# NVlabs/WarpConvNet

Measured on AMD Instinct MI355X. Metric: M active voxels/sec fwd+bwd, SparseConv3d 64→128 k=3, 1/2/4/8 MI355X, higher is better.
Workload: dtype bf16; 1 GPU; configs[1]: one 1000000-voxel uniform (U) scene per GPU, SparseConv3d 64->128 k=3, bf16 autocast, kernel-map build + AB fwd + ABt dgrad + AtB wgrad per step; voxels_per_gpu=1000000, coord_order=generator, parallelism=dp1 (scene-sharded, grad all-reduce)

## Files before the change

warpconvnet_amd/csrc/kmap_binned.hip:

```cpp
#include "kmap_cells.h"

namespace wcn {

constexpr int kInsertSample = 8;
constexpr int kInsertThreads = 512;
constexpr int kRowBufPitch = 66;
constexpr int kRowBufInts = (kCompactPitch + 1) * kRowBufPitch;
#ifndef WCN_NB_WPE
#define WCN_NB_WPE 3
#endif
constexpr int kNbWavesPerSimd = WCN_NB_WPE;
constexpr int kNbThreads = 256;

__device__ __forceinline__ int wrap_blk(int v) {
  const int bits = kBlkCoordBits;
  v &= (1 << bits) - 1;
  return (v ^ (1 << (bits - 1))) - (1 << (bits - 1));
}

__global__ void cell_prepare_kernel(uint4* __restrict__ slots, int64_t capacity, int32_t* __restrict__ ctr,
                                    uint32_t* __restrict__ halo, CellGeom g, int32_t* __restrict__ status) {
  const int64_t i = (int64_t)blockIdx.x * blockDim.x + threadIdx.x;
  if (i < capacity) slots[i] = make_uint4(0u, 0u, 0xFFFFFFFFu, 0u);
  if (i < 64) ctr[i] = 0;
  if (i == 0) *status = 0;
  if (i < g.halo_cells) {
    const int h3[3] = {g.hx, g.hy, g.hz};
    int t = (int)i, dir = 0;
    int sx = 0, sy = 0, sz = 0;
    for (; dir < 27; ++dir) {
      if (dir == 13) continue;
      const int dd[3] = {dir / 9 - 1, (dir / 3) % 3 - 1, dir % 3 - 1};
      sx = dd[0] ? h3[0] : kBlk; sy = dd[1] ? h3[1] : kBlk; sz = dd[2] ? h3[2] : kBlk;
      const int cells = sx * sy * sz;
      if (t < cells) break;
      t -= cells;
    }
    const int ddx = dir / 9 - 1, ddy = (dir / 3) % 3 - 1, ddz = dir % 3 - 1;
    const int tz = t % sz, ty = (t / sz) % sy, tx = t / (sz * sy);
    const int lx = ddx < 0 ? kBlk - g.hx + tx : tx;
    const int ly = ddy < 0 ? kBlk - g.hy + ty : ty;
    const int lz = ddz < 0 ? kBlk - g.hz + tz : tz;
    const int X = lx + kBlk * ddx + g.hx, Y = ly + kBlk * ddy + g.hy, Z = lz + kBlk * ddz + g.hz;
    halo[i] = ((uint32_t)dir << 27) | ((uint32_t)cell_index(lx, ly, lz) << 16) | (uint32_t)(X * g.px + Y * g.py + Z);
  }
}

__device__ __forceinline__ void store_cell(int32_t* cell, int row, bool strict) {
  if (strict) __hip_atomic_fetch_min(reinterpret_cast<uint32_t*>(cell), (uint32_t)row, __ATOMIC_RELAXED, __HIP_MEMORY_SCOPE_AGENT);
  else *cell = row;
}

template <int PHASE>
__global__ __launch_bounds__(kInsertThreads) void cell_insert_kernel(BSlot* __restrict__ slots, uint32_t cmask,
                                                          const int4* __restrict__ coords, int64_t n, CellTable t,
                                                          int32_t* __restrict__ status, int kp, int mw,
                                                          int32_t* __restrict__ nbr, uint32_t* __restrict__ mask,
                                                          int strict) {
  const bool compact = kp < 0;
  kp &= 0x7FFFFFFF;
  const int64_t tid = (int64_t)blockIdx.x * blockDim.x + threadIdx.x;
  const int64_t i = PHASE == 0 ? tid * kInsertSample : tid;
  const int lane = threadIdx.x & 63;
  bool live = i < n;
  int4 c = make_int4(0, 0, 0, 0);
  if (live) {
    c = coords[i];
    if (!coord_in_range(c.x, c.y, c.z, c.w)) {
      live = false;
      if (PHASE == 1) {
        atomicOr(status, (int)WCN_FLAG_COORD_RANGE);
        for (int k = 0; k < kp; ++k) nbr[i * kp + k] = compact ? 0 : -1;
        for (int w = 0; w < mw; ++w) mask[i * mw + w] = 0u;
      }
    }
  }
  int found = -1;
  int id = -1;
  bool created = false;
  uint64_t key = 0;
  if (live) {
    key = pack_key(c.x, c.y >> kBlkShift, c.z >> kBlkShift, c.w >> kBlkShift);
    uint32_t s = hash_slot(key, cmask);
    int idv = -1;
    for (uint32_t a = 0; a <= cmask; ++a) {
      unsigned long long* kptr = reinterpret_cast<unsigned long long*>(&slots[s].key);
      const uint4 v = *reinterpret_cast<const uint4*>(slots + s);
      unsigned long long cur = ((unsigned long long)v.y << 32) | v.x;
      if (cur == key) { found = (int)s; idv = (int)v.z; break; }
      if (cur == 0ull) {
        if (PHASE == 1) cur = __hip_atomic_load(kptr, __ATOMIC_RELAXED, __HIP_MEMORY_SCOPE_AGENT);
        if (cur == 0ull) {
          cur = atomicCAS(kptr, 0ull, (unsigned long long)key);
          if (cur == 0ull) {
            created = true;
            found = (int)s;
            break;
          }
        }
        if (cur == key) { found = (int)s; break; }
      }
      s = (s + 1) & cmask;
    }
    if (found < 0) atomicOr(status, (int)WCN_FLAG_TABLE_FULL);
    if (PHASE == 1 && idv >= 0 && !(idv & kIdLateBit)) id = idv;
  }
  __shared__ int s_made[kInsertThreads / 64 + 1];
  const int wave = threadIdx.x >> 6;
  const unsigned long long makers = __ballot(created);
  if (PHASE == 0) {
    if (lane == 0) s_made[wave] = __popcll(makers);
    __syncthreads();
    if (threadIdx.x == 0) {
      int tot = 0;
      for (int w = 0; w < kInsertThreads / 64; ++w) {
        const int c = s_made[w];
        s_made[w] = tot;
        tot += c;
      }
      s_made[kInsertThreads / 64] = tot > 0 ? atomicAdd(&t.ctr[0], tot) : 0;
    }
    __syncthreads();
  }
  if (makers != 0ull) {
    int base;
    if (PHASE == 0) {
      base = s_made[kInsertThreads / 64] + s_made[wave];
    } else {
      const int leader = __ffsll((long long)makers) - 1;
      base = 0;
      if (lane == leader) base = atomicAdd(&t.ctr[0], __popcll(makers));
      base = __shfl(base, leader);
    }
    int my_id = base + __popcll(makers & ((1ull << lane) - 1ull));
    if (!created) my_id = -1;
    if (my_id >= t.max_blocks) {
      atomicOr(status, (int)WCN_FLAG_TABLE_FULL);
      my_id = -1;
    }
    if (my_id >= 0) {
      t.blk_key[my_id] = key;
      slots[found].id = my_id | (PHASE == 1 ? kIdLateBit : 0);
    }
    unsigned long long todo = makers;
    while (todo != 0ull) {
      const int src = __ffsll((long long)todo) - 1;
      todo &= todo - 1ull;
      const int bid = __shfl(my_id, src);
      if (bid >= 0) {
        int4* gcells = reinterpret_cast<int4*>(t.cells + (int64_t)bid * kCells);
        gcells[lane] = make_int4(-1, -1, -1, -1);
        gcells[lane + 64] = make_int4(-1, -1, -1, -1);
      }
    }
  }
  if (PHASE == 0) return;
  if (live) mask[i * mw + (mw - 1)] = (id >= 0 || found < 0) ? kMaskUnwritten : kMaskDeferred;
  if (id >= 0) store_cell(t.cells + (int64_t)id * kCells + cell_of(c), (int)i, strict != 0);
}

__global__ __launch_bounds__(256) void cell_finish_kernel(const BSlot* __restrict__ slots, uint32_t cmask,
                                                          const int4* __restrict__ coords, int64_t n, CellTable t,
                                                          CellGeom g, int mw, const uint32_t* __restrict__ mask,
                                                          int strict) {
  const int64_t tid = (int64_t)blockIdx.x * blockDim.x + threadIdx.x;
  const int64_t nthreads = (int64_t)gridDim.x * blockDim.x;
  for (int64_t i = tid; i < n; i += nthreads) {
    if (mask[i * mw + (mw - 1)] != kMaskDeferred) continue;
    const int4 c = coords[i];
    const int id = block_id_of(slots, cmask, c);
    if (id < 0) continue;
    store_cell(t.cells + (int64_t)id * kCells + cell_of(c), (int)i, strict != 0);
  }
  const int lane = threadIdx.x & 63;
  int nblocks = t.ctr[0];
  if (nblocks > t.max_blocks) nblocks = (int)t.max_blocks;
  for (int64_t seq = tid >> 6; seq < nblocks; seq += nthreads >> 6) {
    const int id = (int)seq;
    int nid = -1;
    if (lane < 27) {
      const int ddx = lane / 9 - 1, ddy = (lane / 3) % 3 - 1, ddz = lane % 3 - 1;
      const bool needed = (ddx == 0 || g.hx > 0) && (ddy == 0 || g.hy > 0) && (ddz == 0 || g.hz > 0);
      if (lane == 13) nid = id;
      else if (needed) {
        const uint64_t key = t.blk_key[id];
        const int b = (int)((key >> 54) & kBatchMask);
        const int bx = wrap_blk((int)((key >> 36) & kCoordMask));
        const int by = wrap_blk((int)((key >> 18) & kCoordMask));
        const int bz = wrap_blk((int)(key & kCoordMask));
        const int s = block_find(slots, cmask, pack_key(b, wrap_blk(bx + ddx), wrap_blk(by + ddy), wrap_blk(bz + ddz)));
        if (s >= 0) {
          nid = slots[s].id;
          if (nid >= 0) nid &= ~kIdLateBit;
        }
      }
    }
    if (lane < 32) t.nbtab[(int64_t)id * 32 + lane] = nid;
  }
}

#ifdef WCN_PROF
__device__ unsigned long long g_bprof[4096 * 12];
#define BSTAMP(i) do { const unsigned long long now_ = wall_clock64(); prof_acc[i] += now_ - prof_prev; prof_prev = now_; } while (0)
#else
#define BSTAMP(i)
#endif

template <int LPR, bool FAST, bool COMPACT>
__global__ __launch_bounds__(kNbThreads) __attribute__((amdgpu_waves_per_eu(kNbWavesPerSimd))) void cell_neighbors_kernel(CellTable t, const uint32_t* __restrict__ halo,
                                                                    CellGeom g, int K, int kp, int mw,
                                                                    int32_t* __restrict__ nbr,
                                                                    uint32_t* __restrict__ mask,
                                                                    int32_t* __restrict__ status) {
  extern __shared__ int s_mem[];
  const int lane = threadIdx.x & 63, wave = threadIdx.x >> 6;
  uint32_t* s_halo = reinterpret_cast<uint32_t*>(s_mem);
  const int rounds = (g.halo_cells + 63) >> 6;
  const bool halo_regs = COMPACT && rounds <= 8;
  const int halo_pad = halo_regs ? 0 : rounds * 64;
  const int per_wave = g.cells + 4 + kCells / 2 + 8 + (COMPACT ? kRowBufInts : 0);
  int* s_grid = s_mem + halo_pad + wave * per_wave;
  unsigned short* s_own = reinterpret_cast<unsigned short*>(s_grid + g.cells + 4);
  const int null_cell = g.cells;
  for (int h = threadIdx.x; h < halo_pad; h += blockDim.x) s_halo[h] = h < g.halo_cells ? halo[h] : 0xFFFFFFFFu;
  if (lane == 0) s_grid[null_cell] = -1;
  __syncthreads();

  int nblocks = t.ctr[0];
  if (nblocks > t.max_blocks) nblocks = (int)t.max_blocks;
  const int gwave = blockIdx.x * (blockDim.x / 64) + wave;
  const int nwaves = gridDim.x * (blockDim.x / 64);
  constexpr int kVoxPerIter = 64 / LPR;
  const int sub = lane % LPR, vsel = lane / LPR;
  const int num_chunks = (kp + LPR - 1) / LPR;
  uint32_t he[8];
#pragma unroll
  for (int u = 0; u < 8; ++u) {
    const int idx = u * 64 + lane;
    uint32_t e = COMPACT && idx < g.halo_cells ? halo[idx] : 0xFFFFFFFFu;
    if (e == 0xFFFFFFFFu) e = (31u << 27) | (uint32_t)(g.cells + 1);
    he[u] = e;
  }
  auto load_head = [&](int seq, int& nb, int4& v0, int4& v1) {
    nb = -1;
    v0 = make_int4(-1, -1, -1, -1);
    v1 = v0;
    if (seq < nblocks) {
      if (lane < 27) nb = t.nbtab[(int64_t)seq * 32 + lane];
      const int4* own = reinterpret_cast<const int4*>(t.cells + (int64_t)seq * kCells) + lane * 2;
      v0 = own[0];
      v1 = own[1];
    }
  };
  int seq = gwave;
  int nb_c, nb_n;
  int4 c0, c1, n0, n1;
  load_head(seq, nb_c, c0, c1);
  load_head(seq + nwaves, nb_n, n0, n1);
  int hv[8];
  auto gather = [&](int nb, int r0) {
#pragma unroll
    for (int u = 0; u < 8; ++u) {
      hv[u] = -1;
      if (r0 + u < rounds) {
        const uint32_t e = s_halo[(r0 + u) * 64 + lane];
        const int nid = __shfl(nb, (int)((e >> 27) & 31u));
        if (e != 0xFFFFFFFFu && nid >= 0) hv[u] = t.cells[(int64_t)nid * kCells + ((e >> 16) & (kCells - 1))];
      }
    }
  };
  int nidv[8];
  auto gather8 = [&](int nb) {
#pragma unroll
    for (int u = 0; u < 8; ++u) nidv[u] = __shfl(nb, (int)(he[u] >> 27));
#pragma unroll
    for (int u = 0; u < 8; ++u)
      if (u < rounds) {
        const int safe = nidv[u] < 0 ? 0 : nidv[u];
        hv[u] = t.cells[(int64_t)safe * kCells + ((he[u] >> 16) & (kCells - 1))];
      }
  };
  auto scatter8 = [&]() {
#pragma unroll
    for (int u = 0; u < 8; ++u)
      if (u < rounds) s_grid[he[u] & 0xFFFFu] = nidv[u] >= 0 ? hv[u] : -1;
  };
  auto scatter_halo = [&](int r0) {
#pragma unroll
    for (int u = 0; u < 8; ++u)
      if (r0 + u < rounds) {
        const uint32_t e = s_halo[(r0 + u) * 64 + lane];
        if (e != 0xFFFFFFFFu) s_grid[e & 0xFFFFu] = hv[u];
      }
  };
  int* s_rows = s_grid + g.cells + 4 + kCells / 2 + 8;
  int pend_row = -1;
  auto flush_rows = [&](int row) {
    __builtin_amdgcn_fence(__ATOMIC_RELEASE, "wavefront");
    __builtin_amdgcn_wave_barrier();
    if (row >= 0) mask[row] = (uint32_t)s_rows[lane];
    const int piece = lane & 3;
    int rid[4];
    int4 v[4];
#pragma unroll
    for (int q = 0; q < 4; ++q) rid[q] = __shfl(row, (lane >> 2) + 16 * q);
#pragma unroll
    for (int q = 0; q < 4; ++q) {
      const int r = (lane >> 2) + 16 * q;
      v[q].x = s_rows[(piece * 4 + 0) * kRowBufPitch + r];
      v[q].y = s_rows[(piece * 4 + 1) * kRowBufPitch + r];
      v[q].z = s_rows[(piece * 4 + 2) * kRowBufPitch + r];
      v[q].w = s_rows[(piece * 4 + 3) * kRowBufPitch + r];
    }
#pragma unroll
    for (int q = 0; q < 4; ++q)
      if (rid[q] >= 0 && __popc((uint32_t)s_rows[(lane >> 2) + 16 * q]) >= 4 * piece) {
        if (FAST)
          *reinterpret_cast<int4*>(reinterpret_cast<char*>(nbr) + (__umul24((uint32_t)rid[q], kCompactPitch * 4u) + (uint32_t)piece * 16u)) = v[q];
        else
          *reinterpret_cast<int4*>(nbr + (int64_t)rid[q] * kCompactPitch + piece * 4) = v[q];
      }
    __builtin_amdgcn_fence(__ATOMIC_ACQUIRE, "wavefront");
    __builtin_amdgcn_wave_barrier();
  };
#ifdef WCN_PROF
  if (lane == 0 && gwave < 4096) g_bprof[gwave * 12 + 9] = wall_clock64();
#endif
  if (seq < nblocks) {
    if (halo_regs) gather8(nb_c);
    else gather(nb_c, 0);
  }
#ifdef WCN_PROF
  unsigned long long prof_prev = wall_clock64(), prof_acc[8] = {0, 0, 0, 0, 0, 0, 0, 0}, prof_blocks = 0;
  const unsigned long long prof_loop0 = prof_prev;
#endif
  for (; seq < nblocks; seq += nwaves) {
    BSTAMP(0);
#ifdef WCN_PROF
    ++prof_blocks;
#endif
    if (halo_regs) scatter8();
    else scatter_halo(0);
    for (int r0 = 8; r0 < rounds; r0 += 8) {
      gather(nb_c, r0);
      scatter_halo(r0);
    }
    BSTAMP(1);
    const int vals[8] = {c0.x, c0.y, c0.z, c0.w, c1.x, c1.y, c1.z, c1.w};
    const int cell0 = ((lane >> 3) + g.hx) * g.px + ((lane & 7) + g.hy) * g.py + g.hz;
    int mine = 0;
#pragma unroll
    for (int z = 0; z < 8; ++z) {
      s_grid[cell0 + z] = vals[z];
      mine += vals[z] >= 0;
    }
    int incl = mine;
#pragma unroll
    for (int d = 1; d < 64; d <<= 1) {
      const int up = __shfl_up(incl, d);
      if (lane >= d) incl += up;
    }
    const int own_cnt = __shfl(incl, 63);
    int at = incl - mine;
#pragma unroll
    for (int z = 0; z < 8; ++z)
      if (vals[z] >= 0) s_own[at++] = (unsigned short)((cell0 + z) * 4);
    if (lane < 2 * kVoxPerIter) s_own[own_cnt + lane] = (unsigned short)(null_cell * 4);
    BSTAMP(4);
    if (COMPACT) {
      flush_rows(pend_row);
      pend_row = -1;
    }
    BSTAMP(5);
    nb_c = nb_n; c0 = n0; c1 = n1;
    if (seq + nwaves < nblocks) {
      if (halo_regs) gather8(nb_c);
      else gather(nb_c, 0);
    }
    BSTAMP(6);
    load_head(seq + 2 * nwaves, nb_n, n0, n1);
    __builtin_amdgcn_fence(__ATOMIC_RELEASE, "wavefront");
    __builtin_amdgcn_wave_barrier();
    BSTAMP(2);
    const char* grid_bytes = reinterpret_cast<const char*>(s_grid);
    if (COMPACT) {
      int delta_lane = 0;
      if (lane < K) {
        const int l = lane % g.kz, j = (lane / g.kz) % g.ky, i = lane / (g.kz * g.ky);
        delta_lane = ((i - g.cx) * g.dx * g.px + (j - g.cy) * g.dy * g.py + (l - g.cz) * g.dz) * 4;
      }
      bool over = false;
      char* rows_bytes = reinterpret_cast<char*>(s_rows);
      const int origin4 = (g.hx * g.px + g.hy * g.py + g.hz) * 4;
      const uint32_t wp0 = (uint32_t)(kRowBufPitch + lane) * 4u, wp_max = (uint32_t)(kCompactPitch * kRowBufPitch + lane) * 4u;
      for (int e0 = 0; e0 < own_cnt; e0 += 64) {
        const bool live = e0 + lane < own_cnt;
        const int cell = live ? (int)s_own[e0 + lane] : origin4;
        const int row = live ? *reinterpret_cast<const int*>(grid_bytes + cell) : -1;
        uint32_t wp = wp0, rev = 0;
        auto answer = [&](int f) {
          *reinterpret_cast<int*>(rows_bytes + wp) = f;
          const uint32_t h = f >= 0 ? 1u : 0u;
          rev = (rev << 1) | h;
          wp = min(wp + h * (uint32_t)(kRowBufPitch * 4), wp_max);
        };
        int k = 0;
        for (; k + 4 <= K; k += 4) {
          int f[4];
#pragma unroll
          for (int u = 0; u < 4; ++u)
            f[u] = *reinterpret_cast<const int*>(grid_bytes + cell + __builtin_amdgcn_readlane(delta_lane, k + u));
#pragma unroll
          for (int u = 0; u < 4; ++u) answer(f[u]);
        }
        for (; k < K; ++k) answer(*reinterpret_cast<const int*>(grid_bytes + cell + __builtin_amdgcn_readlane(delta_lane, k)));
        const uint32_t m = __brev(rev) >> (32 - K);
        over = over || (live && __popc(m) > kCompactIds);
        s_rows[lane] = (int)m;
        if (e0 + 64 < own_cnt) flush_rows(row);
        else pend_row = row;
      }
      if (__any(over) && lane == 0) atomicOr(status, (int)WCN_FLAG_ROW_OVERFLOW);
    } else
    for (int kc = 0; kc < num_chunks; ++kc) {
      const int k = kc * LPR + sub;
      const bool k_real = k < K, k_store = k < kp;
      const int l = k % g.kz, j = (k / g.kz) % g.ky, i = k / (g.kz * g.ky);
      const int ox = (i - g.cx) * g.dx, oy = (j - g.cy) * g.dy, oz = (l - g.cz) * g.dz;
      const int delta4 = k_real ? (ox * g.px + oy * g.py + oz) * 4 : 0;
      const int w0 = (kc * LPR) >> 5;
      for (int e0 = 0; e0 < own_cnt; e0 += 2 * kVoxPerIter) {
        const int cell_a = s_own[e0 + vsel], cell_b = s_own[e0 + kVoxPerIter + vsel];
        const int row_a = *reinterpret_cast<const int*>(grid_bytes + cell_a);
        const int row_b = *reinterpret_cast<const int*>(grid_bytes + cell_b);
        int found_a = *reinterpret_cast<const int*>(grid_bytes + cell_a + delta4);
        int found_b = *reinterpret_cast<const int*>(grid_bytes + cell_b + delta4);
        if (!k_real) { found_a = -1; found_b = -1; }
        const unsigned long long ball_a = __ballot(found_a >= 0), ball_b = __ballot(found_b >= 0);
        uint32_t bits_a, bits_b, hi_a = 0, hi_b = 0;
        if (LPR == 64) {
          bits_a = (uint32_t)ball_a; hi_a = (uint32_t)(ball_a >> 32);
          bits_b = (uint32_t)ball_b; hi_b = (uint32_t)(ball_b >> 32);
        } else if (LPR == 32) {
          bits_a = vsel ? (uint32_t)(ball_a >> 32) : (uint32_t)ball_a;
          bits_b = vsel ? (uint32_t)(ball_b >> 32) : (uint32_t)ball_b;
        } else {
          bits_a = (uint32_t)(ball_a >> (vsel * LPR)) & ((1u << LPR) - 1u);
          bits_b = (uint32_t)(ball_b >> (vsel * LPR)) & ((1u << LPR) - 1u);
        }
        if (FAST) {
          char* nbr_b = reinterpret_cast<char*>(nbr);
          char* mask_b = reinterpret_cast<char*>(mask);
          const uint32_t kp4 = (uint32_t)kp * 4u, mw4 = (uint32_t)mw * 4u, k4 = (uint32_t)k * 4u, w4 = (uint32_t)w0 * 4u;
          if (row_a >= 0 && k_store) *reinterpret_cast<int*>(nbr_b + (__umul24((uint32_t)row_a, kp4) + k4)) = found_a;
          if (row_b >= 0 && k_store) *reinterpret_cast<int*>(nbr_b + (__umul24((uint32_t)row_b, kp4) + k4)) = found_b;
          if (sub == 0 && w0 < mw) {
            if (row_a >= 0) *reinterpret_cast<uint32_t*>(mask_b + (__umul24((uint32_t)row_a, mw4) + w4)) = bits_a;
            if (row_b >= 0) *reinterpret_cast<uint32_t*>(mask_b + (__umul24((uint32_t)row_b, mw4) + w4)) = bits_b;
            if (LPR == 64 && w0 + 1 < mw) {
              if (row_a >= 0) *reinterpret_cast<uint32_t*>(mask_b + (__umul24((uint32_t)row_a, mw4) + w4 + 4u)) = hi_a;
              if (row_b >= 0) *reinterpret_cast<uint32_t*>(mask_b + (__umul24((uint32_t)row_b, mw4) + w4 + 4u)) = hi_b;
            }
          }
        } else {
          if (row_a >= 0 && k_store) nbr[(int64_t)row_a * kp + k] = found_a;
          if (row_b >= 0 && k_store) nbr[(int64_t)row_b * kp + k] = found_b;
          if (sub == 0 && w0 < mw) {
            if (row_a >= 0) mask[(int64_t)row_a * mw + w0] = bits_a;
            if (row_b >= 0) mask[(int64_t)row_b * mw + w0] = bits_b;
            if (LPR == 64 && w0 + 1 < mw) {
              if (row_a >= 0) mask[(int64_t)row_a * mw + w0 + 1] = hi_a;
              if (row_b >= 0) mask[(int64_t)row_b * mw + w0 + 1] = hi_b;
            }
          }
        }
      }
    }
    BSTAMP(3);

    __builtin_amdgcn_fence(__ATOMIC_ACQUIRE, "wavefront");
    __builtin_amdgcn_wave_barrier();
  }
  if (COMPACT) flush_rows(pend_row);
#ifdef WCN_PROF
  if (lane == 0 && gwave < 4096) {
    for (int i = 0; i < 8; ++i) g_bprof[gwave * 12 + i] = prof_acc[i];
    g_bprof[gwave * 12 + 8] = prof_blocks;
    g_bprof[gwave * 12 + 10] = prof_loop0;
    g_bprof[gwave * 12 + 11] = wall_clock64();
  }
#endif
}

static void launch_cell_table(const CellTable& t, const CellGeom& g, const int4* coords, int64_t n, int kp, int mw, int32_t* nbr,
                              uint32_t* mask, int32_t* status, int strict, hipStream_t s) {
  const int64_t capacity = t.capacity;
  const uint32_t cmask = (uint32_t)(capacity - 1);
  const int64_t max_blocks = t.max_blocks;
  const int64_t prep = capacity > g.halo_cells ? capacity : g.halo_cells;
  hipLaunchKernelGGL(cell_prepare_kernel, dim3((unsigned)ceil_div(prep, 256)), dim3(256), 0, s, (uint4*)t.slots, capacity,
                     t.ctr, t.halo, g, status);
  const int64_t n_first = ceil_div(n, kInsertSample);
  hipLaunchKernelGGL(cell_insert_kernel<0>, dim3((unsigned)ceil_div(n_first, kInsertThreads)), dim3(kInsertThreads), 0, s, t.slots, cmask,
                     coords, n, t, status, kp, mw, nbr, mask, strict);
  hipLaunchKernelGGL(cell_insert_kernel<1>, dim3((unsigned)ceil_div(n, kInsertThreads)), dim3(kInsertThreads), 0, s, t.slots, cmask,
                     coords, n, t, status, kp, mw, nbr, mask, strict);
  {
    const int64_t work = n > 64 * max_blocks ? n : 64 * max_blocks;
    int64_t wgs = ceil_div(work, 256);
    if (wgs > 8192) wgs = 8192;
    hipLaunchKernelGGL(cell_finish_kernel, dim3((unsigned)wgs), dim3(256), 0, s, (const BSlot*)t.slots, cmask,
                       coords, n, t, g, mw, (const uint32_t*)mask, strict);
  }
}

}

using namespace wcn;

extern "C" {

size_t wcn_kmap_binned_workspace(int64_t n, int64_t max_blocks) {
  if (n < 0) n = 0;
  if (max_blocks < 1) max_blocks = 1;
  return carve_cells(nullptr, n, max_blocks).bytes;
}

int wcn_kmap_binned_supported(const int32_t ksize[3], const int32_t dilation[3]) {
  if (!ksize || !dilation) return 0;
  for (int d = 0; d < 3; ++d) {
    if (ksize[d] < 1 || dilation[d] < 1) return 0;
  }
  const int32_t unit[3] = {1, 1, 1};
  const KernelGeom g = make_kernel_geom(ksize, unit, dilation);
  if (kernel_halo(g.kx, g.cx, g.dx) > kMaxHalo || kernel_halo(g.ky, g.cy, g.dy) > kMaxHalo ||
      kernel_halo(g.kz, g.cz, g.dz) > kMaxHalo)
    return 0;
  const int64_t K = (int64_t)ksize[0] * ksize[1] * ksize[2];
  return (valid_k(K) && (K & 31) != 0) ? 1 : 0;
}

int wcn_kmap_compact_supported(int32_t num_offsets) {
  return (num_offsets >= 17 && num_offsets <= 31) ? 1 : 0;
}

int wcn_kmap_build_binned(const int32_t* coords, int64_t n, const int32_t ksize[3], const int32_t dilation[3],
                          int64_t max_blocks, int32_t strict, int32_t compact, void* workspace, size_t workspace_bytes,
                          int32_t* nbr, uint32_t* mask, int32_t* status, wcn_stream_t stream) {
  if (n < 0 || !status || max_blocks < 1 || max_blocks > (1ll << 29)) return WCN_ERROR_INVALID_PARAMETERS;
  if (!wcn_kmap_binned_supported(ksize, dilation)) return WCN_ERROR_PROBLEM_NOT_SUPPORTED;
  if (compact && (!ksize || !wcn_kmap_compact_supported(ksize[0] * ksize[1] * ksize[2]))) return WCN_ERROR_PROBLEM_NOT_SUPPORTED;
  if (n == 0) return WCN_SUCCESS;
  if (n >= (1ll << 31) || !coords || !nbr || !mask || !workspace ||
      workspace_bytes < wcn_kmap_binned_workspace(n, max_blocks))
    return WCN_ERROR_INVALID_PARAMETERS;
  hipStream_t s = (hipStream_t)stream;
  const CellTable t = carve_cells(workspace, n, max_blocks);
  const int K = ksize[0] * ksize[1] * ksize[2];
  const int kp = wcn_kmap_row_pitch(K), mw = wcn_kmap_mask_words(K);
  const CellGeom g = make_cell_geom(ksize, dilation);
  const int64_t capacity = t.capacity;
  const uint32_t cmask = (uint32_t)(capacity - 1);

  launch_cell_table(t, g, (const int4*)coords, n, compact ? (kCompactPitch | kCompactFlag) : kp, mw, nbr, mask, status, (int)strict, s);
  const int halo_rounds = (g.halo_cells + 63) >> 6;
  const int halo_pad = compact && halo_rounds <= 8 ? 0 : halo_rounds * 64;
  int nb_waves = kNbThreads / 64;
  auto shm_for = [&](int waves) {
    return ((size_t)halo_pad + (size_t)waves * (g.cells + 4 + kCells / 2 + 8 + (compact ? kRowBufInts : 0))) * 4;
  };
  while (nb_waves > 1 && shm_for(nb_waves) > 156 * 1024) nb_waves >>= 1;
  const size_t shm = shm_for(nb_waves);
  if (shm > 160 * 1024) return WCN_ERROR_PROBLEM_NOT_SUPPORTED;
  int per_cu = (int)((160 * 1024) / (shm + 512));
  if (per_cu > 8) per_cu = 8;
  if (compact && per_cu * nb_waves > 4 * kNbWavesPerSimd) per_cu = 4 * kNbWavesPerSimd / nb_waves;
  if (per_cu < 1) per_cu = 1;
  int64_t want = ceil_div(max_blocks < n ? max_blocks : n, nb_waves);
  if (want > 256 * per_cu) want = 256 * per_cu;
  const dim3 grid((unsigned)want), block(nb_waves * 64);
  if (shm > 64 * 1024) {
    static unsigned long long attr_done = 0ull;
    const int rc = once_per_device(attr_done, [] {
      bool ok = true;
      for (const void* f : {reinterpret_cast<const void*>(cell_neighbors_kernel<8, true, false>), reinterpret_cast<const void*>(cell_neighbors_kernel<8, false, false>),
                            reinterpret_cast<const void*>(cell_neighbors_kernel<16, true, false>), reinterpret_cast<const void*>(cell_neighbors_kernel<16, false, false>),
                            reinterpret_cast<const void*>(cell_neighbors_kernel<32, true, false>), reinterpret_cast<const void*>(cell_neighbors_kernel<32, false, false>),
                            reinterpret_cast<const void*>(cell_neighbors_kernel<32, true, true>), reinterpret_cast<const void*>(cell_neighbors_kernel<32, false, true>),
                            reinterpret_cast<const void*>(cell_neighbors_kernel<64, true, false>), reinterpret_cast<const void*>(cell_neighbors_kernel<64, false, false>)})
        ok = ok && hipFuncSetAttribute(f, hipFuncAttributeMaxDynamicSharedMemorySize, 160 * 1024) == hipSuccess;
      return ok;
    });
    if (rc != WCN_SUCCESS) return rc;
  }
  const bool fast = n < (1ll << 24) && n * kp * 4 < (1ll << 31);
#define WCN_CELL_NB(L, C)                                                                                                 \
  do {                                                                                                                    \
    if (fast)                                                                                                             \
      hipLaunchKernelGGL((cell_neighbors_kernel<L, true, C>), grid, block, shm, s, t, (const uint32_t*)t.halo, g, K, kp,  \
                         mw, nbr, mask, status);                                                                          \
    else                                                                                                                  \
      hipLaunchKernelGGL((cell_neighbors_kernel<L, false, C>), grid, block, shm, s, t, (const uint32_t*)t.halo, g, K, kp, \
                         mw, nbr, mask, status);                                                                          \
  } while (0)
  if (compact) {
    WCN_CELL_NB(32, true);
  } else {
    switch (lanes_per_row(kp)) {
      case 8: WCN_CELL_NB(8, false); break;
      case 16: WCN_CELL_NB(16, false); break;
      case 32: WCN_CELL_NB(32, false); break;
      default: WCN_CELL_NB(64, false); break;
    }
  }
#undef WCN_CELL_NB
  return launch_status();
}

int wcn_kmap_cells_build(const int32_t* coords, int64_t n, int64_t max_blocks, void* workspace, size_t workspace_bytes,
                         uint32_t* scratch, int32_t* status, wcn_stream_t stream) {
  if (n < 0 || !status || max_blocks < 1 || max_blocks > (1ll << 29)) return WCN_ERROR_INVALID_PARAMETERS;
  if (n == 0) return WCN_SUCCESS;
  if (n >= (1ll << 31) || !coords || !scratch || !workspace || workspace_bytes < wcn_kmap_binned_workspace(n, max_blocks))
    return WCN_ERROR_INVALID_PARAMETERS;
  const CellTable t = carve_cells(workspace, n, max_blocks);
  const int32_t one[3] = {1, 1, 1};
  const CellGeom g = make_cell_geom(one, one);
  launch_cell_table(t, g, (const int4*)coords, n, 0, 1, nullptr, scratch, status, 1, (hipStream_t)stream);
  return launch_status();
}

}

#ifdef WCN_PROF
extern "C" int wcn_debug_read_bprof(void* dst, size_t bytes) {
  return (int)hipMemcpyFromSymbol(dst, HIP_SYMBOL(wcn::g_bprof), bytes);
}
#endif
```

warpconvnet_amd/csrc/kmap_cells.h:

```cpp
#pragma once

#include "wcn_common.h"

namespace wcn {

constexpr int kBlkShift = 3;
constexpr int kBlk = 1 << kBlkShift;
constexpr int kCells = kBlk * kBlk * kBlk;
constexpr int kMaxHalo = 8;
constexpr int kBlkCoordBits = kCoordBits - kBlkShift;
constexpr uint32_t kMaskUnwritten = 0x80000000u;
constexpr uint32_t kMaskDeferred = 0x80000001u;

constexpr int kCompactPitch = 16;
constexpr int kCompactIds = kCompactPitch - 1;
constexpr int kCompactFlag = (int)0x80000000;

constexpr int kIdLateBit = 1 << 30;

struct __attribute__((aligned(16))) BSlot {
  uint64_t key;
  int32_t id;
  int32_t pad;
};

struct CellTable {
  BSlot* slots;
  int64_t capacity;
  int32_t* ctr;
  uint32_t* halo;
  uint64_t* blk_key;
  int32_t* nbtab;
  int32_t* cells;
  int64_t max_blocks;
  size_t bytes;
};

struct KernelGeom {
  int kx, ky, kz;
  int cx, cy, cz;
  int sx, sy, sz;
  int dx, dy, dz;
};

static inline KernelGeom make_kernel_geom(const int32_t ksize[3], const int32_t stride[3], const int32_t dilation[3]) {
  auto centre = [](int ks) { return (ks & 1) ? ks / 2 : 0; };
  return KernelGeom{ksize[0],  ksize[1],  ksize[2],  centre(ksize[0]), centre(ksize[1]), centre(ksize[2]),
                    stride[0], stride[1], stride[2], dilation[0],      dilation[1],      dilation[2]};
}

static inline int kernel_halo(int ks, int c, int d) {
  const int lo = c * d, hi = (ks - 1 - c) * d;
  return lo > hi ? lo : hi;
}

static inline int lanes_per_row(int kp) {
  int l = 8;
  while (l < kp && l < 64) l <<= 1;
  return l;
}

struct CellGeom {
  int kx, ky, kz, cx, cy, cz, dx, dy, dz;
  int hx, hy, hz;
  int px, py;
  int cells;
  int halo_cells;
};

static inline int64_t cell_capacity(int64_t max_blocks) {
  int64_t c = 1024;
  while (c < 2 * max_blocks) c <<= 1;
  return c;
}

static inline CellTable carve_cells(void* ws, int64_t n, int64_t max_blocks) {
  CellTable t;
  char* p = (char*)ws;
  size_t off = 0;
  auto take = [&](size_t bytes) { char* q = p ? p + off : nullptr; off += align256(bytes); return q; };
  (void)n;
  t.max_blocks = max_blocks;
  t.capacity = cell_capacity(max_blocks);
  t.ctr = (int32_t*)take(256);
  t.halo = (uint32_t*)take((size_t)16384 * 4);
  t.slots = (BSlot*)take((size_t)t.capacity * sizeof(BSlot));
  t.blk_key = (uint64_t*)take((size_t)max_blocks * 8);
  t.nbtab = (int32_t*)take((size_t)max_blocks * 32 * 4);
  t.cells = (int32_t*)take((size_t)max_blocks * kCells * 4);
  t.bytes = off;
  return t;
}

static inline CellGeom make_cell_geom(const int32_t ksize[3], const int32_t dilation[3]) {
  const int32_t unit[3] = {1, 1, 1};
  const KernelGeom k = make_kernel_geom(ksize, unit, dilation);
  CellGeom g;
  g.kx = k.kx; g.ky = k.ky; g.kz = k.kz;
  g.cx = k.cx; g.cy = k.cy; g.cz = k.cz;
  g.dx = k.dx; g.dy = k.dy; g.dz = k.dz;
  g.hx = kernel_halo(g.kx, g.cx, g.dx); g.hy = kernel_halo(g.ky, g.cy, g.dy); g.hz = kernel_halo(g.kz, g.cz, g.dz);
  const int gx = kBlk + 2 * g.hx, gy = kBlk + 2 * g.hy, gz = kBlk + 2 * g.hz;
  g.py = gz | 1;
  g.px = gy * g.py;
  g.cells = gx * g.px;
  g.halo_cells = gx * gy * gz - kCells;
  return g;
}

__device__ __forceinline__ int block_find(const BSlot* __restrict__ slots, uint32_t cmask, uint64_t key) {
  uint32_t s = hash_slot(key, cmask);
  for (uint32_t a = 0; a <= cmask; ++a) {
    const uint64_t k = slots[s].key;
    if (k == 0ull) return -1;
    if (k == key) return (int)s;
    s = (s + 1) & cmask;
  }
  return -1;
}

__device__ __forceinline__ int block_id_of(const BSlot* __restrict__ slots, uint32_t cmask, const int4& c) {
  const int s = block_find(slots, cmask, pack_key(c.x, c.y >> kBlkShift, c.z >> kBlkShift, c.w >> kBlkShift));
  if (s < 0) return -1;
  const int id = slots[s].id;
  return id < 0 ? -1 : (id & ~kIdLateBit);
}

__device__ __forceinline__ int cell_index(int x, int y, int z) { return (x * kBlk + y) * kBlk + z; }
__device__ __forceinline__ int cell_of(const int4& c) {
  return ((c.y & (kBlk - 1)) * kBlk + (c.z & (kBlk - 1))) * kBlk + (c.w & (kBlk - 1));
}

}
```

Baseline: 1081 M voxels/s.

## Add dense bounding-box direct block indexing to kernel-map build

The prepare kernel now computes a per-batch bounding box of coordinate blocks. When the box is dense enough, block IDs are assigned directly from box position instead of by hash insertion, neighbour tables are filled arithmetically, and the finish pass is skipped. Separately, in direct mode the neighbour kernel assigns contiguous runs of blocks to each group of workgroups (grouped by blockIdx mod 8), meant to improve locality per XCD. This adds a box reduction and extra prepare work, and falls back to hashing when the scene is sparse.

```diff
diff --git a/warpconvnet_amd/csrc/kmap_binned.hip b/warpconvnet_amd/csrc/kmap_binned.hip
--- a/warpconvnet_amd/csrc/kmap_binned.hip
+++ b/warpconvnet_amd/csrc/kmap_binned.hip
@@ -4,12 +4,19 @@
 
 constexpr int kInsertSample = 8;
 constexpr int kInsertThreads = 512;
+constexpr int kPrepThreads = 1024;
+constexpr int kPrepCoordsPerPart = 4096;
+constexpr int kDirectMaxGrid = 1024;
 constexpr int kRowBufPitch = 66;
 constexpr int kRowBufInts = (kCompactPitch + 1) * kRowBufPitch;
 #ifndef WCN_NB_WPE
 #define WCN_NB_WPE 3
 #endif
 constexpr int kNbWavesPerSimd = WCN_NB_WPE;
+#ifndef WCN_NB_XCD_RUNS
+#define WCN_NB_XCD_RUNS 1
+#endif
+constexpr bool kNbXcdRuns = WCN_NB_XCD_RUNS != 0;
 constexpr int kNbThreads = 256;
 
 __device__ __forceinline__ int wrap_blk(int v) {
@@ -18,9 +25,45 @@
   return (v ^ (1 << (bits - 1))) - (1 << (bits - 1));
 }
 
-__global__ void cell_prepare_kernel(uint4* __restrict__ slots, int64_t capacity, int32_t* __restrict__ ctr,
-                                    uint32_t* __restrict__ halo, CellGeom g, int32_t* __restrict__ status) {
+__global__ __launch_bounds__(kPrepThreads) void cell_prepare_kernel(uint4* __restrict__ slots, int64_t capacity, int32_t* __restrict__ ctr,
+                                    uint32_t* __restrict__ halo, CellGeom g, int32_t* __restrict__ status,
+                                    const int4* __restrict__ coords, int64_t n, int parts, int32_t* __restrict__ box) {
   const int64_t i = (int64_t)blockIdx.x * blockDim.x + threadIdx.x;
+  if ((int)blockIdx.x < parts) {
+    __shared__ int s_box[kPrepThreads / 64][8];
+    int m[8];
+#pragma unroll
+    for (int a = 0; a < 8; ++a) m[a] = INT_MAX;
+    const int64_t step = (int64_t)parts * kPrepThreads;
+    for (int64_t j = i; j < n; j += 4 * step) {
+      int4 c[4];
+#pragma unroll
+      for (int u = 0; u < 4; ++u) c[u] = coords[j + u * step < n ? j + u * step : j];
+#pragma unroll
+      for (int u = 0; u < 4; ++u) {
+        if (!coord_in_range(c[u].x, c[u].y, c[u].z, c[u].w)) continue;
+        const int v[4] = {c[u].x, c[u].y >> kBlkShift, c[u].z >> kBlkShift, c[u].w >> kBlkShift};
+#pragma unroll
+        for (int a = 0; a < 4; ++a) {
+          m[a] = min(m[a], v[a]);
+          m[4 + a] = min(m[4 + a], -v[a]);
+        }
+      }
+    }
+#pragma unroll
+    for (int d = 1; d < 64; d <<= 1)
+#pragma unroll
+      for (int a = 0; a < 8; ++a) m[a] = min(m[a], __shfl_xor(m[a], d));
+    if ((threadIdx.x & 63) == 0)
+#pragma unroll
+      for (int a = 0; a < 8; ++a) s_box[threadIdx.x >> 6][a] = m[a];
+    __syncthreads();
+    if (threadIdx.x < 8) {
+      int r = INT_MAX;
+      for (int w = 0; w < kPrepThreads / 64; ++w) r = min(r, s_box[w][threadIdx.x]);
+      box[blockIdx.x * 8 + threadIdx.x] = r;
+    }
+  }
   if (i < capacity) slots[i] = make_uint4(0u, 0u, 0xFFFFFFFFu, 0u);
   if (i < 64) ctr[i] = 0;
   if (i == 0) *status = 0;
@@ -51,17 +94,95 @@
   else *cell = row;
 }
 
+
+__device__ __forceinline__ BlockBox reduce_box(const int32_t* __restrict__ box, int parts) {
+  __shared__ __attribute__((aligned(16))) int s_red[kInsertThreads / 64][8];
+  int v = INT_MAX;
+  for (int j = threadIdx.x; j < parts * 8; j += kInsertThreads) v = min(v, box[j]);
+  v = min(v, __shfl_xor(v, 8));
+  v = min(v, __shfl_xor(v, 16));
+  v = min(v, __shfl_xor(v, 32));
+  if ((threadIdx.x & 63) < 8) s_red[threadIdx.x >> 6][threadIdx.x & 7] = v;
+  __syncthreads();
+  int lo[4] = {INT_MAX, INT_MAX, INT_MAX, INT_MAX}, nhi[4] = {INT_MAX, INT_MAX, INT_MAX, INT_MAX};
+#pragma unroll
+  for (int w = 0; w < kInsertThreads / 64; ++w) {
+    const int4 a = *reinterpret_cast<const int4*>(&s_red[w][0]), b = *reinterpret_cast<const int4*>(&s_red[w][4]);
+    lo[0] = min(lo[0], a.x); lo[1] = min(lo[1], a.y); lo[2] = min(lo[2], a.z); lo[3] = min(lo[3], a.w);
+    nhi[0] = min(nhi[0], b.x); nhi[1] = min(nhi[1], b.y); nhi[2] = min(nhi[2], b.z); nhi[3] = min(nhi[3], b.w);
+  }
+  const int hi[4] = {-nhi[0], -nhi[1], -nhi[2], -nhi[3]};
+  return make_block_box(lo, hi);
+}
+
+__device__ __forceinline__ void direct_blocks(BSlot* __restrict__ slots, uint32_t cmask, const CellTable& t, const BlockBox& box,
+                                              int nblocks, int hx, int hy, int hz, int32_t* __restrict__ status) {
+  const int lane = threadIdx.x & 63;
+  const int nwaves = gridDim.x * (kInsertThreads / 64);
+  const int ddx = lane / 9 - 1, ddy = (lane / 3) % 3 - 1, ddz = lane % 3 - 1;
+  const bool needed = lane < 27 && (ddx == 0 || hx > 0) && (ddy == 0 || hy > 0) && (ddz == 0 || hz > 0);
+  for (int id = blockIdx.x * (kInsertThreads / 64) + (threadIdx.x >> 6); id < nblocks; id += nwaves) {
+    int r[4];
+    box_block_pos(box, id, r);
+    int4* gcells = reinterpret_cast<int4*>(t.cells + (int64_t)id * kCells);
+    gcells[lane] = make_int4(-1, -1, -1, -1);
+    gcells[lane + 64] = make_int4(-1, -1, -1, -1);
+    if (lane < 32) t.nbtab[(int64_t)id * 32 + lane] = needed ? box_block_id(box, r[0], r[1] + ddx, r[2] + ddy, r[3] + ddz) : -1;
+    if (lane == 0) {
+      const uint64_t key = box_block_key(box, r);
+      t.blk_key[id] = key;
+      uint32_t s = hash_slot(key, cmask);
+      bool placed = false;
+      for (uint32_t a = 0; a <= cmask && !placed; ++a) {
+        if (atomicCAS(reinterpret_cast<unsigned long long*>(&slots[s].key), 0ull, (unsigned long long)key) == 0ull) {
+          slots[s].id = id;
+          placed = true;
+        }
+        s = (s + 1) & cmask;
+      }
+      if (!placed) atomicOr(status, (int)WCN_FLAG_TABLE_FULL);
+    }
+  }
+  if (blockIdx.x == 0 && threadIdx.x == 0) {
+    t.ctr[kCtrBlocks] = nblocks;
+    t.ctr[kCtrMode] = 1;
+    for (int a = 0; a < 4; ++a) {
+      t.ctr[kCtrBox + a] = box.o[a];
+      t.ctr[kCtrBox + 4 + a] = box.d[a];
+    }
+  }
+}
+
 template <int PHASE>
 __global__ __launch_bounds__(kInsertThreads) void cell_insert_kernel(BSlot* __restrict__ slots, uint32_t cmask,
                                                           const int4* __restrict__ coords, int64_t n, CellTable t,
                                                           int32_t* __restrict__ status, int kp, int mw,
                                                           int32_t* __restrict__ nbr, uint32_t* __restrict__ mask,
-                                                          int strict) {
+                                                          int strict, int box_parts, int halo3) {
   const bool compact = kp < 0;
   kp &= 0x7FFFFFFF;
   const int64_t tid = (int64_t)blockIdx.x * blockDim.x + threadIdx.x;
   const int64_t i = PHASE == 0 ? tid * kInsertSample : tid;
   const int lane = threadIdx.x & 63;
+  bool direct = false;
+  BlockBox box = {};
+  if (PHASE == 0) {
+    if (box_parts > 0) {
+      box = reduce_box(t.box, box_parts);
+      if (box_is_direct(box, n, t.max_blocks)) {
+        direct_blocks(slots, cmask, t, box, (int)box_blocks(box), halo3 & 255, (halo3 >> 8) & 255, (halo3 >> 16) & 255, status);
+        return;
+      }
+    }
+    if ((int64_t)blockIdx.x * kInsertThreads * kInsertSample >= n) return;
+  } else {
+    direct = t.ctr[kCtrMode] != 0;
+#pragma unroll
+    for (int a = 0; a < 4; ++a) {
+      box.o[a] = t.ctr[kCtrBox + a];
+      box.d[a] = t.ctr[kCtrBox + 4 + a];
+    }
+  }
   bool live = i < n;
   int4 c = make_int4(0, 0, 0, 0);
   if (live) {
@@ -79,7 +200,11 @@
   int id = -1;
   bool created = false;
   uint64_t key = 0;
-  if (live) {
+  if (live && direct) {
+    id = box_block_id(box, c.x - box.o[0], (c.y >> kBlkShift) - box.o[1], (c.z >> kBlkShift) - box.o[2], (c.w >> kBlkShift) - box.o[3]);
+    if (id < 0) atomicOr(status, (int)WCN_FLAG_TABLE_FULL);
+  }
+  if (live && !direct) {
     key = pack_key(c.x, c.y >> kBlkShift, c.z >> kBlkShift, c.w >> kBlkShift);
     uint32_t s = hash_slot(key, cmask);
     int idv = -1;
@@ -163,6 +288,7 @@
                                                           const int4* __restrict__ coords, int64_t n, CellTable t,
                                                           CellGeom g, int mw, const uint32_t* __restrict__ mask,
                                                           int strict) {
+  if (t.ctr[kCtrMode] != 0) return;
   const int64_t tid = (int64_t)blockIdx.x * blockDim.x + threadIdx.x;
   const int64_t nthreads = (int64_t)gridDim.x * blockDim.x;
   for (int64_t i = tid; i < n; i += nthreads) {
@@ -230,6 +356,13 @@
   if (nblocks > t.max_blocks) nblocks = (int)t.max_blocks;
   const int gwave = blockIdx.x * (blockDim.x / 64) + wave;
   const int nwaves = gridDim.x * (blockDim.x / 64);
+  int first = gwave, stride = nwaves, end = nblocks;
+  if (kNbXcdRuns && gridDim.x >= 8 && t.ctr[kCtrMode] != 0) {
+    const int grp = blockIdx.x & 7, members = (gridDim.x - grp + 7) >> 3;
+    first = (int)(((int64_t)nblocks * grp) >> 3) + (blockIdx.x >> 3) * (blockDim.x / 64) + wave;
+    stride = members * (blockDim.x / 64);
+    end = (int)(((int64_t)nblocks * (grp + 1)) >> 3);
+  }
   constexpr int kVoxPerIter = 64 / LPR;
   const int sub = lane % LPR, vsel = lane / LPR;
   const int num_chunks = (kp + LPR - 1) / LPR;
@@ -245,18 +378,18 @@
     nb = -1;
     v0 = make_int4(-1, -1, -1, -1);
     v1 = v0;
-    if (seq < nblocks) {
+    if (seq < end) {
       if (lane < 27) nb = t.nbtab[(int64_t)seq * 32 + lane];
       const int4* own = reinterpret_cast<const int4*>(t.cells + (int64_t)seq * kCells) + lane * 2;
       v0 = own[0];
       v1 = own[1];
     }
   };
-  int seq = gwave;
+  int seq = first;
   int nb_c, nb_n;
   int4 c0, c1, n0, n1;
   load_head(seq, nb_c, c0, c1);
-  load_head(seq + nwaves, nb_n, n0, n1);
+  load_head(seq + stride, nb_n, n0, n1);
   int hv[8];
   auto gather = [&](int nb, int r0) {
 #pragma unroll
@@ -326,7 +459,7 @@
 #ifdef WCN_PROF
   if (lane == 0 && gwave < 4096) g_bprof[gwave * 12 + 9] = wall_clock64();
 #endif
-  if (seq < nblocks) {
+  if (seq < end) {
     if (halo_regs) gather8(nb_c);
     else gather(nb_c, 0);
   }
@@ -334,7 +467,7 @@
   unsigned long long prof_prev = wall_clock64(), prof_acc[8] = {0, 0, 0, 0, 0, 0, 0, 0}, prof_blocks = 0;
   const unsigned long long prof_loop0 = prof_prev;
 #endif
-  for (; seq < nblocks; seq += nwaves) {
+  for (; seq < end; seq += stride) {
     BSTAMP(0);
 #ifdef WCN_PROF
     ++prof_blocks;
@@ -373,12 +506,12 @@
     }
     BSTAMP(5);
     nb_c = nb_n; c0 = n0; c1 = n1;
-    if (seq + nwaves < nblocks) {
+    if (seq + stride < end) {
       if (halo_regs) gather8(nb_c);
       else gather(nb_c, 0);
     }
     BSTAMP(6);
-    load_head(seq + 2 * nwaves, nb_n, n0, n1);
+    load_head(seq + 2 * stride, nb_n, n0, n1);
     __builtin_amdgcn_fence(__ATOMIC_RELEASE, "wavefront");
     __builtin_amdgcn_wave_barrier();
     BSTAMP(2);
@@ -492,19 +625,36 @@
 #endif
 }
 
+static bool direct_mode_enabled() {
+  const char* e = getenv("WARPCONVNET_AMD_KMAP_DIRECT");
+  return !(e && e[0] == '0' && e[1] == '\0');
+}
+
 static void launch_cell_table(const CellTable& t, const CellGeom& g, const int4* coords, int64_t n, int kp, int mw, int32_t* nbr,
                               uint32_t* mask, int32_t* status, int strict, hipStream_t s) {
   const int64_t capacity = t.capacity;
   const uint32_t cmask = (uint32_t)(capacity - 1);
   const int64_t max_blocks = t.max_blocks;
-  const int64_t prep = capacity > g.halo_cells ? capacity : g.halo_cells;
-  hipLaunchKernelGGL(cell_prepare_kernel, dim3((unsigned)ceil_div(prep, 256)), dim3(256), 0, s, (uint4*)t.slots, capacity,
-                     t.ctr, t.halo, g, status);
+  const bool try_direct = direct_mode_enabled();
+  int64_t parts = try_direct ? ceil_div(n, kPrepCoordsPerPart) : 0;
+  if (parts > kBoxParts) parts = kBoxParts;
+  int64_t prep = ceil_div(capacity > g.halo_cells ? capacity : g.halo_cells, kPrepThreads);
+  if (prep < parts) prep = parts;
+  hipLaunchKernelGGL(cell_prepare_kernel, dim3((unsigned)prep), dim3(kPrepThreads), 0, s, (uint4*)t.slots, capacity,
+                     t.ctr, t.halo, g, status, coords, n, (int)parts, t.box);
   const int64_t n_first = ceil_div(n, kInsertSample);
-  hipLaunchKernelGGL(cell_insert_kernel<0>, dim3((unsigned)ceil_div(n_first, kInsertThreads)), dim3(kInsertThreads), 0, s, t.slots, cmask,
-                     coords, n, t, status, kp, mw, nbr, mask, strict);
+  int64_t first_wgs = ceil_div(n_first, kInsertThreads);
+  if (try_direct) {
+    const int64_t most = max_blocks < n / kDirectFill ? max_blocks : n / kDirectFill;
+    int64_t want = ceil_div(most, kInsertThreads / 64);
+    if (want > kDirectMaxGrid) want = kDirectMaxGrid;
+    if (first_wgs < want) first_wgs = want;
+  }
+  const int halo3 = g.hx | (g.hy << 8) | (g.hz << 16);
+  hipLaunchKernelGGL(cell_insert_kernel<0>, dim3((unsigned)first_wgs), dim3(kInsertThreads), 0, s, t.slots, cmask,
+                     coords, n, t, status, kp, mw, nbr, mask, strict, (int)parts, halo3);
   hipLaunchKernelGGL(cell_insert_kernel<1>, dim3((unsigned)ceil_div(n, kInsertThreads)), dim3(kInsertThreads), 0, s, t.slots, cmask,
-                     coords, n, t, status, kp, mw, nbr, mask, strict);
+                     coords, n, t, status, kp, mw, nbr, mask, strict, 0, halo3);
   {
     const int64_t work = n > 64 * max_blocks ? n : 64 * max_blocks;
     int64_t wgs = ceil_div(work, 256);
diff --git a/warpconvnet_amd/csrc/kmap_cells.h b/warpconvnet_amd/csrc/kmap_cells.h
--- a/warpconvnet_amd/csrc/kmap_cells.h
+++ b/warpconvnet_amd/csrc/kmap_cells.h
@@ -24,10 +24,64 @@
   int32_t pad;
 };
 
+constexpr int kCtrBlocks = 0;
+constexpr int kCtrMode = 1;
+constexpr int kCtrBox = 2;
+
+constexpr int kDirectFill = 16;
+constexpr int kBoxParts = 128;
+
+struct BlockBox {
+  int o[4];
+  int d[4];
+};
+
+__host__ __device__ inline BlockBox make_block_box(const int lo[4], const int hi[4]) {
+  BlockBox b;
+  const bool empty = lo[0] > hi[0];
+  for (int a = 0; a < 4; ++a) {
+    b.o[a] = empty ? 0 : lo[a];
+    b.d[a] = empty ? 0 : hi[a] - lo[a] + 1;
+  }
+  return b;
+}
+
+__host__ __device__ inline int64_t box_blocks(const BlockBox& b) {
+  return (int64_t)b.d[0] * b.d[1] * b.d[2] * b.d[3];
+}
+
+__host__ __device__ inline bool box_is_direct(const BlockBox& b, int64_t n, int64_t max_blocks) {
+  const int64_t blocks = box_blocks(b);
+  if (blocks < 1 || blocks > max_blocks || blocks > n / kDirectFill) return false;
+  const int lo = -(1 << (kBlkCoordBits - 1)), hi = (1 << (kBlkCoordBits - 1)) - 1;
+  for (int a = 1; a < 4; ++a)
+    if (b.o[a] <= lo || b.o[a] + b.d[a] - 1 >= hi) return false;
+  return true;
+}
+
+__host__ __device__ inline int box_block_id(const BlockBox& b, int r0, int r1, int r2, int r3) {
+  if ((unsigned)r0 >= (unsigned)b.d[0] || (unsigned)r1 >= (unsigned)b.d[1] || (unsigned)r2 >= (unsigned)b.d[2] ||
+      (unsigned)r3 >= (unsigned)b.d[3])
+    return -1;
+  return ((r0 * b.d[1] + r1) * b.d[2] + r2) * b.d[3] + r3;
+}
+
+__host__ __device__ inline void box_block_pos(const BlockBox& b, int id, int r[4]) {
+  r[3] = id % b.d[3]; id /= b.d[3];
+  r[2] = id % b.d[2]; id /= b.d[2];
+  r[1] = id % b.d[1];
+  r[0] = id / b.d[1];
+}
+
+__host__ __device__ inline uint64_t box_block_key(const BlockBox& b, const int r[4]) {
+  return pack_key(b.o[0] + r[0], b.o[1] + r[1], b.o[2] + r[2], b.o[3] + r[3]);
+}
+
 struct CellTable {
   BSlot* slots;
   int64_t capacity;
   int32_t* ctr;
+  int32_t* box;
   uint32_t* halo;
   uint64_t* blk_key;
   int32_t* nbtab;
@@ -83,6 +137,7 @@
   t.max_blocks = max_blocks;
   t.capacity = cell_capacity(max_blocks);
   t.ctr = (int32_t*)take(256);
+  t.box = (int32_t*)take((size_t)kBoxParts * 8 * 4);
   t.halo = (uint32_t*)take((size_t)16384 * 4);
   t.slots = (BSlot*)take((size_t)t.capacity * sizeof(BSlot));
   t.blk_key = (uint64_t*)take((size_t)max_blocks * 8);
```

Result: faster. 1113 M voxels/s (median of 6 runs) (+3.0%).
